# HarborC/PL-SLAM

Measured on NVIDIA H100. Metric: frames/sec (extract+match+pose-LM) 640x480, higher is better.
Workload: dtype u8/i32 front-end, f32 descriptors, f64 LM

## Files before the change

### pl-slam_b200/csrc/line.cu

```cuda

#include "common.cuh"
#include "lsd_grow_core.cuh"
#include "libm_glibc.cuh"
#include <math.h>
#include <string.h>
#include <stdlib.h>
#include <vector>
#include <algorithm>

namespace pl {

constexpr double kPI = 3.14159265358979323846;
constexpr double kDegToRads = kPI / 180;
constexpr int kBins = 1024;
constexpr int kChunkRows = 8;


struct PLKeyLineRec {
  float angle; int class_id; int octave; float ptx, pty; float response; float size;
  float startPointX, startPointY, endPointX, endPointY;
  float sPointInOctaveX, sPointInOctaveY, ePointInOctaveX, ePointInOctaveY;
  float lineLength; int numOfPixels;
};
static_assert(sizeof(PLKeyLineRec) == 68, "KeyLine layout");

struct LineParams {
  int w, h, sw, sh, npx;
  int nchunk;
  int s_th;
  int min_reg_size;
  int seg_cap, capL, nfeatures;
  double min_line_length;
  double prec, prec_hi, p, density_th;
  float sure_ca2, sure_cn2;
};

__device__ __forceinline__ float fast_atan2_deg_l(float y, float x) {
  const float k = (float)(180.0 / 3.14159265358979323846);
  const float p1 = 0.9997878412794807f * k, p3 = -0.3258083974640975f * k;
  const float p5 = 0.1555786518463281f * k, p7 = -0.04432655554792128f * k;
  const float eps = 2.220446049250313e-16f;
  const float ax = fabsf(x), ay = fabsf(y);
  const float c = __fdiv_rn(fminf(ax, ay), __fadd_rn(fmaxf(ax, ay), eps)), c2 = __fmul_rn(c, c);
  float a = __fmul_rn(__fadd_rn(__fmul_rn(__fadd_rn(__fmul_rn(__fadd_rn(__fmul_rn(p7, c2), p5), c2), p3), c2), p1), c);
  if (ax < ay) a = __fsub_rn(90.f, a);
  if (x < 0) a = __fsub_rn(180.f, a);
  if (y < 0) a = __fsub_rn(360.f, a);
  return a;
}
__device__ __forceinline__ double warp_max_d(double v) {
#pragma unroll
  for (int o = 16; o > 0; o >>= 1) v = fmax(v, __shfl_xor_sync(0xffffffffu, v, o));
  return v;
}
__device__ __forceinline__ double warp_min_d(double v) {
#pragma unroll
  for (int o = 16; o > 0; o >>= 1) v = fmin(v, __shfl_xor_sync(0xffffffffu, v, o));
  return v;
}

__global__ void __launch_bounds__(256) k_lsd_scale(LineParams P, const uint8_t* __restrict__ imgs, int stride,
                                                   long long frame_stride, uint8_t* __restrict__ scaled) {
  __shared__ uint8_t raw[44][48];
  __shared__ uint16_t hp[44][40];
  __shared__ uint8_t bl[40][40];
  const int tid = threadIdx.x;
  const int X0 = blockIdx.x * 32, Y0 = blockIdx.y * 32;
  const int bx0 = (5 * X0) >> 2, by0 = (5 * Y0) >> 2;
  const uint8_t* img = imgs + (long long)blockIdx.z * frame_stride;
  for (int i = tid; i < 44 * 44; i += 256) {
    int r = i / 44, c = i - r * 44;
    int gy = reflect101(min(by0 - 2 + r, 2 * P.h - 2), P.h), gx = reflect101(min(bx0 - 2 + c, 2 * P.w - 2), P.w);
    raw[r][c] = img[(long long)gy * stride + gx];
  }
  __syncthreads();
  for (int i = tid; i < 44 * 40; i += 256) {
    int r = i / 40, c = i - r * 40;
    const uint8_t* p = &raw[r][c];
    hp[r][c] = (uint16_t)(4 * (p[0] + p[4]) + 56 * (p[1] + p[3]) + 136 * p[2]);
  }
  __syncthreads();
  for (int i = tid; i < 40 * 40; i += 256) {
    int r = i / 40, c = i - r * 40;
    uint32_t s = 4u * (hp[r][c] + hp[r + 4][c]) + 56u * (hp[r + 1][c] + hp[r + 3][c]) + 136u * hp[r + 2][c];
    bl[r][c] = (uint8_t)((s + 32768u) >> 16);
  }
  __syncthreads();
  uint8_t* out = scaled + (long long)blockIdx.z * P.npx;
  for (int i = tid; i < 32 * 32; i += 256) {
    int ty = i >> 5, tx = i & 31;
    int x = X0 + tx, y = Y0 + ty;
    if (x >= P.sw || y >= P.sh) continue;
    int sx = (10 * x + 1) >> 3, xf = ((10 * x + 1) & 7) * 32;
    int sy = (10 * y + 1) >> 3, yf = ((10 * y + 1) & 7) * 32;
    if (sx >= P.w - 1) { sx = P.w - 1; xf = 0; }
    if (sy >= P.h - 1) { sy = P.h - 1; yf = 0; }
    int sx1 = min(sx + 1, P.w - 1), sy1 = min(sy + 1, P.h - 1);
    int lx = sx - bx0, lx1 = sx1 - bx0, ly = sy - by0, ly1 = sy1 - by0;
    int h0 = bl[ly][lx] * (256 - xf) + bl[ly][lx1] * xf;
    int h1 = bl[ly1][lx] * (256 - xf) + bl[ly1][lx1] * xf;
    out[(long long)y * P.sw + x] = (uint8_t)((h0 * (256 - yf) + h1 * yf + 32768) >> 16);
  }
}

constexpr float kNotDefDeg = -1024.f;
constexpr int kGradR = 510, kGradN = 2 * kGradR + 1;
struct GradRec { float deg, c, s, pad; };
__device__ __forceinline__ void grad_record(int gx, int gy, GradRec& rec, float2& scs) {
  const float deg = fast_atan2_deg_l((float)gx, (float)(-gy));
  const double af = (double)(float)((double)deg * kDegToRads);
  double sn, cs;
  sincos(af, &sn, &cs);
  rec.deg = deg; rec.c = (float)cs; rec.s = (float)sn; rec.pad = 0.f;
  const double ad = (double)deg * kDegToRads, dl = ad - af, h2 = 1.0 - 0.5 * dl * dl;
  scs = make_float2((float)(cs * h2 - sn * dl), (float)(sn * h2 + cs * dl));
}
__global__ void __launch_bounds__(256) k_lsd_grad_table(GradRec* __restrict__ T, float2* __restrict__ TS) {
  const int i = blockIdx.x * blockDim.x + threadIdx.x;
  if (i >= kGradN * kGradN) return;
  GradRec rec; float2 scs;
  grad_record(i / kGradN - kGradR, i % kGradN - kGradR, rec, scs);
  T[i] = rec; TS[i] = scs;
}
template <bool kVec>
__global__ void __launch_bounds__(256) k_lsd_grad(LineParams P, const uint8_t* __restrict__ scaled, const float4* __restrict__ T,
                                                  const float2* __restrict__ TS,
                                                  int4* __restrict__ REC, int* __restrict__ S2, float2* __restrict__ seedcs, int* __restrict__ maxs) {
  __shared__ int smax;
  if (threadIdx.x == 0) smax = 0;
  __syncthreads();
  const int x0 = (blockIdx.x * 64 + (threadIdx.x & 63)) * 4, y = blockIdx.y * 4 + (threadIdx.x >> 6);
  const int f = blockIdx.z;
  int smx = 0;
  if (x0 < P.sw && y < P.sh) {
    const uint8_t* S = scaled + (long long)f * P.npx + (long long)y * P.sw + x0;
    const bool lastrow = (y >= P.sh - 1);
    int r0[5], r1[5];
    if (kVec) {
      const unsigned w0 = *reinterpret_cast<const unsigned*>(S), w1 = lastrow ? 0u : *reinterpret_cast<const unsigned*>(S + P.sw);
#pragma unroll
      for (int k = 0; k < 4; k++) { r0[k] = (w0 >> (8 * k)) & 0xff; r1[k] = (w1 >> (8 * k)) & 0xff; }
      const bool in4 = (x0 + 4 < P.sw);
      r0[4] = in4 ? S[4] : 0; r1[4] = (in4 && !lastrow) ? S[P.sw + 4] : 0;
    } else {
#pragma unroll
      for (int k = 0; k < 5; k++) {
        const bool in = (x0 + k < P.sw);
        r0[k] = in ? S[k] : 0;
        r1[k] = (in && !lastrow) ? S[P.sw + k] : 0;
      }
    }
    int4 rec[4];
    float se[4][2];
    int sq[4];
#pragma unroll
    for (int k = 0; k < 4; k++) {
      rec[k] = make_int4(lg::kNotDef, __float_as_int(kNotDefDeg), 0, 0); se[k][0] = se[k][1] = 0.f; sq[k] = 0;
      if (x0 + k < P.sw - 1 && !lastrow) {
        const int DA = r1[k + 1] - r0[k], BC = r0[k + 1] - r1[k];
        const int gx = DA + BC, gy = DA - BC;
        const int s = gx * gx + gy * gy;
        sq[k] = s;
        if (s > P.s_th) {
          const int ti = (gx + kGradR) * kGradN + (gy + kGradR);
          const float4 t = __ldg(&T[ti]);
          const float2 scs = __ldg(&TS[ti]);
          rec[k] = make_int4(lg::kFree, __float_as_int(t.x), __float_as_int(t.y), __float_as_int(t.z));
          se[k][0] = scs.x; se[k][1] = scs.y;
          smx = max(smx, s);
        }
      }
    }
    const long long o = (long long)f * P.npx + (long long)y * P.sw + x0;
    if (kVec) {
#pragma unroll
      for (int k = 0; k < 4; k++) REC[o + k] = rec[k];
      *reinterpret_cast<int4*>(S2 + o) = make_int4(sq[0], sq[1], sq[2], sq[3]);
      float4* e4 = reinterpret_cast<float4*>(seedcs + o);
      e4[0] = make_float4(se[0][0], se[0][1], se[1][0], se[1][1]); e4[1] = make_float4(se[2][0], se[2][1], se[3][0], se[3][1]);
    } else {
      for (int k = 0; k < 4 && x0 + k < P.sw; k++) { REC[o + k] = rec[k]; S2[o + k] = sq[k]; seedcs[o + k] = make_float2(se[k][0], se[k][1]); }
    }
  }
#pragma unroll
  for (int o = 16; o > 0; o >>= 1) smx = max(smx, __shfl_xor_sync(0xffffffffu, smx, o));
  if ((threadIdx.x & 31) == 0 && smx > 0) atomicMax(&smax, smx);
  __syncthreads();
  if (threadIdx.x == 0 && smax > 0) atomicMax(&maxs[f], smax);
}
__device__ __forceinline__ double s_norm(int s) { return sqrt((double)s / 4.0); }
__device__ __forceinline__ int s_bin(int s, double bin_coef) { return (int)(s_norm(s) * bin_coef); }

__global__ void __launch_bounds__(256) k_lsd_hist(LineParams P, const int* __restrict__ S2, const int* __restrict__ maxs,
                                                  unsigned short* __restrict__ counts ) {
  __shared__ int hist[kBins];
  const int chunk = blockIdx.x, f = blockIdx.y, tid = threadIdx.x;
  for (int i = tid; i < kBins; i += 256) hist[i] = 0;
  __syncthreads();
  const int ms = maxs[f];
  const double max_grad = ms > 0 ? sqrt((double)ms / 4.0) : -1.0;
  const double bin_coef = (max_grad > 0) ? (double)(kBins - 1) / max_grad : 0.0;
  const int y0 = chunk * kChunkRows, y1 = min(y0 + kChunkRows, P.sh - 1);
  const int* SS = S2 + (long long)f * P.npx;
  for (int i = tid; i < (y1 - y0) * P.sw; i += 256) {
    int y = y0 + i / P.sw, x = i % P.sw;
    const int sv = SS[y * P.sw + x];
    if (sv > P.s_th) atomicAdd(&hist[s_bin(sv, bin_coef)], 1);
  }
  __syncthreads();
  for (int i = tid; i < kBins; i += 256) counts[((long long)f * kBins + i) * P.nchunk + chunk] = (unsigned short)hist[i];
}

__global__ void __launch_bounds__(kBins) k_lsd_scan(LineParams P, const unsigned short* __restrict__ counts,
                                                    int* __restrict__ offsets, int* __restrict__ ndef) {
  __shared__ int wsum[32];
  const int f = blockIdx.x, t = threadIdx.x, bin = kBins - 1 - t, lane = t & 31, wid = t >> 5;
  const unsigned short* c = counts + ((long long)f * kBins + bin) * P.nchunk;
  int tot = 0;
  for (int k = 0; k < P.nchunk; k++) tot += c[k];
  int incl = tot;
#pragma unroll
  for (int o = 1; o < 32; o <<= 1) { int v = __shfl_up_sync(0xffffffffu, incl, o); if (lane >= o) incl += v; }
  if (lane == 31) wsum[wid] = incl;
  __syncthreads();
  if (wid == 0) {
    int v = wsum[lane], in2 = v;
#pragma unroll
    for (int o = 1; o < 32; o <<= 1) { int u = __shfl_up_sync(0xffffffffu, in2, o); if (lane >= o) in2 += u; }
    wsum[lane] = in2 - v;
    if (lane == 31) ndef[f] = in2;
  }
  __syncthreads();
  int base = wsum[wid] + incl - tot;
  int* o = offsets + ((long long)f * kBins + bin) * P.nchunk;
  for (int k = 0; k < P.nchunk; k++) { o[k] = base; base += c[k]; }
}

__global__ void __launch_bounds__(128) k_lsd_scatter(LineParams P, const int* __restrict__ S2, const int* __restrict__ maxs,
                                                     const int* __restrict__ offsets, unsigned* __restrict__ order) {
  __shared__ unsigned short cnt[4][kBins];
  const int wid = threadIdx.x >> 5, lane = threadIdx.x & 31;
  const int chunk = blockIdx.x * 4 + wid, f = blockIdx.y;
  for (int i = lane; i < kBins; i += 32) cnt[wid][i] = 0;
  __syncwarp();
  if (chunk >= P.nchunk) return;
  const int ms = maxs[f];
  const double max_grad = ms > 0 ? sqrt((double)ms / 4.0) : -1.0;
  const double bin_coef = (max_grad > 0) ? (double)(kBins - 1) / max_grad : 0.0;
  const int y0 = chunk * kChunkRows, y1 = min(y0 + kChunkRows, P.sh - 1);
  const int* SS = S2 + (long long)f * P.npx;
  const int* off = offsets + (long long)f * kBins * P.nchunk;
  unsigned* O = order + (long long)f * P.npx;
  const int n = (y1 - y0) * P.sw;
  const unsigned lt = (1u << lane) - 1u;
  for (int i0 = 0; i0 < n; i0 += 32) {
    int i = i0 + lane, bin = -1, pix = 0;
    if (i < n) {
      int y = y0 + i / P.sw, x = i % P.sw;
      pix = x | (y << 16);
      const int sv = SS[y * P.sw + x];
      if (sv > P.s_th) bin = s_bin(sv, bin_coef);
    }
    unsigned peers = __match_any_sync(0xffffffffu, bin);
    if (bin >= 0) O[off[bin * P.nchunk + chunk] + cnt[wid][bin] + __popc(peers & lt)] = (unsigned)pix;
    __syncwarp();
    if (bin >= 0 && (peers & lt) == 0) cnt[wid][bin] += (unsigned short)__popc(peers);
    __syncwarp();
  }
}

constexpr int kGrowQ = 256;
constexpr int kCommitBatches = 4;
constexpr unsigned kGrowWatchdog = 6u * 1000u * 1000u;
__device__ __forceinline__ int first_zero(unsigned m) { return m == 0xffffffffu ? 32 : __ffs(~m) - 1; }

__device__ __forceinline__ void warp_commit(const lg::Params& GP, const lg::Frame& Fm, float4* __restrict__ segs, int lane) {
  using namespace lg;
  const unsigned lt = (1u << lane) - 1u;
  for (int round = 0; round < kCommitBatches; round++) {
    const int F = ld_i(&Fm.ctl[C_FIN]);
    if (F >= Fm.n) return;
    const int i = F + lane;
    const unsigned w1 = (i < Fm.n) ? ld_u(&Fm.st[i]) : 0u;
    const unsigned s1 = w1 & ST_STATE;
    const int pre1 = first_zero(__ballot_sync(0xffffffffu, s1 == ST_NOOP || s1 == ST_EATEN || s1 == ST_DONE));
    if (pre1 == 0) return;
    __threadfence();
    unsigned w2 = 0u;
    bool ok = false;
    if (lane < pre1) { w2 = ld_u(&Fm.st[i]); ok = task_valid(GP, Fm, i, w2); }
    const int pre2 = min(pre1, first_zero(__ballot_sync(0xffffffffu, ok)));
    float4 sg;
    const bool has = (lane < pre2) && task_has_segment(Fm, w2, sg);
    const unsigned ms = __ballot_sync(0xffffffffu, has);
    const int ns = ld_i(&Fm.ctl[C_NS]);
    if (has) { const int slot = ns + __popc(ms & lt); if (slot < GP.seg_cap) segs[slot] = sg; }
    __syncwarp();
    if (lane == 0) {
      st_i(&Fm.ctl[C_NS], ns + __popc(ms));
      __threadfence();
      a_max(&Fm.ctl[C_FIN], F + pre2);
    }
    if (pre2 < pre1) {
      const unsigned s2 = w2 & ST_STATE;
      if (lane == pre2 && (s2 == ST_DONE || s2 == ST_EATEN) &&
          (unsigned)a_cas(reinterpret_cast<int*>(&Fm.st[i]), (int)w2, (int)((w2 & ~(ST_STATE | ST_ABORT)) | ST_REDO)) == w2) {
        __threadfence();
        st_i(&Fm.ctl[C_REDO], i);
      }
      __syncwarp();
      return;
    }
    __syncwarp();
    if (pre2 < 32) return;
  }
}

template <int kWPC>
__global__ void __launch_bounds__(32 * kWPC) k_lsd_grow(LineParams P, lg::Params GP, int4* __restrict__ REC, const float2* __restrict__ seedcs,
                                                        const int* __restrict__ SQ, const unsigned* __restrict__ order, const int* __restrict__ ndef,
                                                        unsigned* __restrict__ ST, unsigned* __restrict__ POOL, int* __restrict__ CTL,
                                                        unsigned* __restrict__ LANEBUF, const double* __restrict__ wtab,
                                                        float4* __restrict__ segs, int* __restrict__ nseg, int* __restrict__ overflow,
                                                        int nframes, int wpf) {
  using namespace lg;
  __shared__ int wq_all[kWPC][kGrowQ];
  __shared__ unsigned ring_all[kWPC][32 * lg::kRing];
  const int lane = threadIdx.x & 31, wic = threadIdx.x >> 5;
  const long long gw = (long long)blockIdx.x * kWPC + wic;
  const int f = (int)(gw / wpf), wif = (int)(gw % wpf);
  if (f >= nframes) return;
  int* wq = wq_all[wic];
  Frame Fm;
  Fm.rec = REC + (long long)f * P.npx; Fm.seedcs = seedcs + (long long)f * P.npx; Fm.sq = SQ + (long long)f * P.npx;
  Fm.order = order + (long long)f * P.npx; Fm.n = ndef[f];
  Fm.st = ST + (long long)f * P.npx; Fm.pool = POOL + (long long)f * GP.pool_cap; Fm.ctl = CTL + (long long)f * kCtlStride; Fm.wtab = wtab;
  float4* S = segs + (long long)f * P.seg_cap;
  const bool solo = (wpf == 1);
  if (!solo && wif == 0) {
    for (unsigned iter = 0;; iter++) {
      __syncwarp();
      const int F = __shfl_sync(0xffffffffu, ld_i(&Fm.ctl[C_FIN]), 0);
      if (F >= Fm.n) break;
      if (iter > 4u * kGrowWatchdog) {
        if (lane == 0) { a_or(reinterpret_cast<unsigned*>(&Fm.ctl[C_ERR]), (unsigned)ERR_WATCHDOG); a_max(&Fm.ctl[C_FIN], Fm.n); }
        break;
      }
      warp_commit(GP, Fm, S, lane);
      if (__shfl_sync(0xffffffffu, ld_i(&Fm.ctl[C_FIN]), 0) == F) __nanosleep(200);
    }
    if (lane == 0) {
// ... 337 lines not shown
      if (gDL > 0) pgdL = __fadd_rn(pgdL, gDL); else ngdL = __fsub_rn(ngdL, gDL);
      if (gDO > 0) pgdO = __fadd_rn(pgdO, gDO); else ngdO = __fsub_rn(ngdO, gDO);
      sCorX = __fadd_rn(sCorX, dL0); sCorY = __fadd_rn(sCorY, dL1);
    }
    const float c = c_gaussG[hID];
    pgdL = __fmul_rn(c, pgdL); ngdL = __fmul_rn(c, ngdL); pgdO = __fmul_rn(c, pgdO); ngdO = __fmul_rn(c, ngdO);
    rs[hID][0] = pgdL; rs[hID][1] = ngdL; rs[hID][2] = __fmul_rn(pgdL, pgdL); rs[hID][3] = __fmul_rn(ngdL, ngdL);
    rs[hID][4] = pgdO; rs[hID][5] = ngdO; rs[hID][6] = __fmul_rn(pgdO, pgdO); rs[hID][7] = __fmul_rn(ngdO, ngdO);
  }
  __syncthreads();
  for (int a = tid; a < 72; a += 64) {
    const int q = a / 9, k = a - q * 9;
    const bool sq = (q == 2 || q == 3 || q == 6 || q == 7);
    float b = 0.f;
    for (int B = max(k - 1, 0); B <= min(k + 1, 8); B++) {
      const int off = (B - k + 1) * 7;
      for (int j = 0; j < 7; j++) {
        const float cg = s_gL[j + off], v = rs[B * 7 + j][q];
        b = __fadd_rn(b, sq ? __fmul_rn(__fmul_rn(cg, cg), v) : __fmul_rn(cg, v));
      }
    }
    band[q][k] = b;
  }
  __syncthreads();
  if (tid < 36) {
    const int bb = tid >> 2, c = tid & 3;
    const int qm = (c & 1) + ((c & 2) << 1), qs = qm + 2;
    const float invN = (bb == 0 || bb == 8) ? (float)(1.0 / (7 * 2.0)) : (float)(1.0 / (7 * 3.0));
    const float temp = __fmul_rn(band[qm][bb], invN);
    des[8 * bb + c] = temp;
    des[8 * bb + 4 + c] = sqrtf(__fsub_rn(__fmul_rn(band[qs][bb], invN), __fmul_rn(temp, temp)));
  }
  __syncthreads();
  if (tid == 0 || tid == 32) {
    const int k0 = tid ? 4 : 0;
    float acc = 0;
    for (int i = 0; i < 72; i += 8)
      for (int k = k0; k < k0 + 4; k++) acc = __fadd_rn(acc, __fmul_rn(des[i + k], des[i + k]));
    s_norm2[tid ? 1 : 0] = __fdiv_rn(1.f, sqrtf(acc));
  }
  __syncthreads();
  for (int i = tid; i < 72; i += 64) {
    float v = __fmul_rn(des[i], s_norm2[(i & 7) >> 2]);
    if ((double)v > 0.4) v = (float)0.4;
    des[i] = v;
  }
  __syncthreads();
  if (tid == 0) {
    float temp = 0;
    for (int i = 0; i < 72; i++) temp = __fadd_rn(temp, __fmul_rn(des[i], des[i]));
    s_norm2[0] = __fdiv_rn(1.f, sqrtf(temp));
  }
  __syncthreads();
  for (int i = tid; i < 72; i += 64) des[i] = __fmul_rn(des[i], s_norm2[0]);
  __syncthreads();
  if (tid < 32) {
    const float* f1 = &des[8 * c_comb[2 * tid]];
    const float* f2 = &des[8 * c_comb[2 * tid + 1]];
    unsigned r = 0;
#pragma unroll
    for (int i = 0; i < 8; i++) if (f1[i] > f2[i]) r += (1u << i);
    desc[((long long)f * P.capL + li) * 32 + tid] = (uint8_t)r;
  }
}

}

using namespace pl;

struct PLLine {
  PLLineConfig cfg;
  LineParams P;
  cudaStream_t stream = nullptr;
  uint8_t* d_scaled = nullptr;
  float2* d_seedcs = nullptr;
  lg::Params GP;
  int grow_warps_target = 132 * 16;
  int grow_wpf_max = 64;
  int grow_spec_max_batch = 0;
  size_t lane_warps = 0;
  int4* d_rec = nullptr; int* d_sq = nullptr;
  unsigned *d_st = nullptr, *d_pool = nullptr, *d_lanebuf = nullptr; int* d_ctl = nullptr; double* d_wtab = nullptr;
  GradRec* d_gtab = nullptr; float2* d_gtab_seed = nullptr;
  unsigned short* d_counts = nullptr;
  int *d_offsets = nullptr, *d_ndef = nullptr, *d_maxs = nullptr, *d_nseg = nullptr, *d_overflow = nullptr;
  unsigned* d_order = nullptr;
  float4* d_segs = nullptr;
  short2* d_dxy = nullptr;
  uint8_t* d_img = nullptr; PLKeyLineRec* d_kls = nullptr; uint8_t* d_desc = nullptr; double* d_lf = nullptr; int* d_nl = nullptr;
  uint8_t* d_mask = nullptr;
  size_t key_smem = 0;
  int last_B = 0;
  int timing = 0;
  cudaEvent_t ev0 = nullptr, ev1 = nullptr;
};

static const unsigned char h_comb[64] = {0, 1, 0, 2, 0, 3, 0, 4, 0, 5, 0, 6, 1, 2, 1, 3, 1, 4, 1, 5, 1, 6, 2, 3, 2, 4, 2, 5, 2, 6, 2, 7,
                                         2, 8, 3, 4, 3, 5, 3, 6, 3, 7, 3, 8, 4, 5, 4, 6, 4, 7, 4, 8, 5, 6, 5, 7, 5, 8, 6, 7, 6, 8, 7, 8};

extern "C" void pl_line_destroy(PLLine* h) {
  if (!h) return;
  cudaFree(h->d_gtab); cudaFree(h->d_gtab_seed); cudaFree(h->d_scaled); cudaFree(h->d_seedcs); cudaFree(h->d_rec); cudaFree(h->d_sq); cudaFree(h->d_st); cudaFree(h->d_pool); cudaFree(h->d_lanebuf); cudaFree(h->d_ctl); cudaFree(h->d_wtab); cudaFree(h->d_counts); cudaFree(h->d_offsets);
  cudaFree(h->d_ndef); cudaFree(h->d_maxs); cudaFree(h->d_nseg); cudaFree(h->d_overflow); cudaFree(h->d_order);
  cudaFree(h->d_segs); cudaFree(h->d_dxy); cudaFree(h->d_img); cudaFree(h->d_kls);
  cudaFree(h->d_desc); cudaFree(h->d_lf); cudaFree(h->d_nl); cudaFree(h->d_mask);
  if (h->stream) cudaStreamDestroy(h->stream);
  delete h;
}

extern "C" int pl_line_create(const PLLineConfig* cfg, PLLine** out) {
  PL_ARG(cfg && out);
  PL_ARG(cfg->width >= 64 && cfg->height >= 64 && cfg->width < 8000 && cfg->height < 8000 && cfg->nfeatures > 0 && cfg->max_batch >= 1);
  int rc = require_device();
  if (rc) return rc;
  PLLine* h = new PLLine;
  h->cfg = *cfg;
  LineParams& P = h->P;
  P.w = cfg->width; P.h = cfg->height;
  P.sw = (int)lrint(P.w * 0.8); P.sh = (int)lrint(P.h * 0.8);
  P.npx = P.sw * P.sh;
  P.nchunk = (P.sh - 1 + kChunkRows - 1) / kChunkRows;
  const double ANG_TH = 22.5, QUANT = 2.0;
  P.prec = kPI * ANG_TH / 180; P.p = ANG_TH / 180; P.density_th = 0.7;
  {
    const double twopi = 2 * kPI;
    double c = twopi - P.prec;
    while ((twopi - nextafter(c, 0.0)) <= P.prec) c = nextafter(c, 0.0);
    while (!((twopi - c) <= P.prec)) c = nextafter(c, 10.0);
    P.prec_hi = c;
  }
  {
    const double M = 0.05 * M_PI / 180.0, ca = cos(P.prec - M), cn = cos(P.prec + M);
    P.sure_ca2 = (float)(ca * ca); P.sure_cn2 = (float)(cn * cn);
  }
  const double rho = QUANT / sin(P.prec);
  int s = 0;
  while (sqrt((double)(s + 1) / 4.0) <= rho) s++;
  P.s_th = s;
  const double LOG_NT = 5 * (log10((double)P.sw) + log10((double)P.sh)) / 2 + log10(11.0);
  P.min_reg_size = (int)(size_t)(-LOG_NT / log10(P.p));
  P.seg_cap = cfg->segment_cap > 0 ? cfg->segment_cap : 8192;
  P.nfeatures = cfg->nfeatures; P.capL = cfg->nfeatures + 1; P.min_line_length = cfg->min_line_length;
  { size_t c2 = 1; while (c2 < (size_t)P.seg_cap) c2 <<= 1; h->key_smem = c2 * 8; }
  const size_t B = cfg->max_batch, npx = P.npx;
#define LN_TRY(e) do { int _r = (e); if (_r) { pl_line_destroy(h); return _r; } } while (0)
#define LN_CUDA(e) do { cudaError_t _e = (e); if (_e != cudaSuccess) { set_error("%s -> %s", #e, cudaGetErrorString(_e)); pl_line_destroy(h); return PL_ERR_CUDA; } } while (0)
  LN_CUDA(cudaStreamCreateWithFlags(&h->stream, cudaStreamNonBlocking));
  LN_TRY(dev_alloc(&h->d_scaled, npx * B)); LN_TRY(dev_alloc(&h->d_seedcs, npx * B)); LN_TRY(dev_alloc(&h->d_rec, npx * B));
  LN_TRY(dev_alloc(&h->d_sq, npx * B));
  {
    int dev = 0, sms = 132;
    cudaGetDevice(&dev); cudaDeviceGetAttribute(&sms, cudaDevAttrMultiProcessorCount, dev);
    h->grow_warps_target = sms * 16;
    if (const char* e = getenv("PLSLAM_LSD_GROW_WARPS")) { const int v = atoi(e); if (v > 0) h->grow_warps_target = v; }
    if (const char* e = getenv("PLSLAM_LSD_GROW_WPF")) { const int v = atoi(e); if (v > 0) h->grow_wpf_max = v; }
    if (const char* e = getenv("PLSLAM_LSD_GROW_SPEC_MAXB")) h->grow_spec_max_batch = atoi(e);
    lg::Params& G = h->GP;
    G.sw = P.sw; G.sh = P.sh; G.npx = P.npx; G.min_reg_size = P.min_reg_size; G.seg_cap = P.seg_cap;
    G.lane_cap = 1024; G.pool_cap = 4 * P.npx; G.window = 8192;
    if (const char* e = getenv("PLSLAM_LSD_GROW_WINDOW")) G.window = atoi(e);
    G.prec = P.prec; G.prec_hi = P.prec_hi; G.density_th = P.density_th;
    h->lane_warps = std::max<size_t>(std::min<size_t>(B * (size_t)h->grow_wpf_max, (size_t)h->grow_warps_target), B);
    LN_TRY(dev_alloc(&h->d_st, npx * B)); LN_TRY(dev_alloc(&h->d_pool, (size_t)G.pool_cap * B)); LN_TRY(dev_alloc(&h->d_ctl, (size_t)lg::kCtlStride * B));
    LN_TRY(dev_alloc(&h->d_lanebuf, h->lane_warps * 32 * (size_t)G.lane_cap));
    const int nw = 2 * kGradR * kGradR + 1;
    LN_TRY(dev_alloc(&h->d_wtab, (size_t)nw));
    k_lsd_wtab<<<(nw + 255) / 256, 256, 0, h->stream>>>(h->d_wtab, nw);
    LN_CUDA(cudaGetLastError());
    count_launch();
  }
  LN_TRY(dev_alloc(&h->d_counts, (size_t)kBins * P.nchunk * B)); LN_TRY(dev_alloc(&h->d_offsets, (size_t)kBins * P.nchunk * B));
  LN_TRY(dev_alloc(&h->d_ndef, B)); LN_TRY(dev_alloc(&h->d_maxs, B)); LN_TRY(dev_alloc(&h->d_nseg, B)); LN_TRY(dev_alloc(&h->d_overflow, 1));
  LN_TRY(dev_alloc(&h->d_order, npx * B)); LN_TRY(dev_alloc(&h->d_segs, (size_t)P.seg_cap * B));
  LN_TRY(dev_alloc(&h->d_dxy, (size_t)P.w * P.h * B));
  LN_CUDA(cudaMemset(h->d_overflow, 0, sizeof(int)));
  LN_TRY(dev_alloc(&h->d_gtab, (size_t)kGradN * kGradN)); LN_TRY(dev_alloc(&h->d_gtab_seed, (size_t)kGradN * kGradN));
  k_lsd_grad_table<<<(kGradN * kGradN + 255) / 256, 256, 0, h->stream>>>(h->d_gtab, h->d_gtab_seed);
  LN_CUDA(cudaGetLastError());
  LN_CUDA(cudaStreamSynchronize(h->stream));
  count_launch();
  {
    float gG[63], gL[21];
    double u = (7 * 3 - 1) / 2, sigma = (7 * 2 + 1) / 2, inv = -1 / (2 * sigma * sigma);
    for (int i = 0; i < 21; i++) { double d = i - u; gL[i] = (float)exp(d * d * inv); }
    u = (9 * 7 - 1) / 2; sigma = u; inv = -1 / (2 * sigma * sigma);
    for (int i = 0; i < 63; i++) { double d = i - u; gG[i] = (float)exp(d * d * inv); }
    LN_CUDA(cudaMemcpyToSymbol(c_gaussG, gG, sizeof(gG)));
    LN_CUDA(cudaMemcpyToSymbol(c_gaussL, gL, sizeof(gL)));
    LN_CUDA(cudaMemcpyToSymbol(c_comb, h_comb, sizeof(h_comb)));
  }
  LN_CUDA(cudaFuncSetAttribute(k_keylines, cudaFuncAttributeMaxDynamicSharedMemorySize, (int)h->key_smem));
  *out = h;
  return PL_OK;
}

extern "C" int pl_line_capacity(const PLLine* h) { return h ? h->P.capL : PL_ERR_ARG; }

extern "C" int pl_line_set_timing(PLLine* h, int on) {
  PL_ARG(h);
  if (on && !h->ev0) { PL_CUDA(cudaEventCreate(&h->ev0)); PL_CUDA(cudaEventCreate(&h->ev1)); }
  h->timing = on;
  return PL_OK;
}
extern "C" int pl_line_grow_ms(PLLine* h, float* ms) {
  PL_ARG(h && ms && h->ev0);
  PL_CUDA(cudaEventSynchronize(h->ev1));
  PL_CUDA(cudaEventElapsedTime(ms, h->ev0, h->ev1));
  return PL_OK;
}
extern "C" long long pl_line_grow_bytes_per_frame(const PLLine* h) { return h ? (long long)h->P.npx * 28 : 0; }

extern "C" int pl_line_extract_batch_dev(PLLine* h, const uint8_t* imgs, int stride, size_t frame_stride, int B,
                                         const uint8_t* mask, void* keylines, uint8_t* desc, double* linefunc, int* n,
                                         void* stream_) {
  PL_ARG(h && imgs && keylines && desc && linefunc && n && B >= 1 && B <= h->cfg.max_batch && stride >= h->cfg.width);
  cudaStream_t st = stream_ ? (cudaStream_t)stream_ : h->stream;
  const LineParams& P = h->P;
  h->last_B = B;
  PL_CUDA(cudaMemsetAsync(h->d_maxs, 0, sizeof(int) * B, st));
  k_lsd_scale<<<dim3((P.sw + 31) / 32, (P.sh + 31) / 32, B), 256, 0, st>>>(P, imgs, stride, (long long)frame_stride, h->d_scaled);
  PL_LAUNCH_CHECK();
  {
    const dim3 grd((P.sw + 255) / 256, (P.sh + 3) / 4, B);
    if (P.sw % 4 == 0)
      k_lsd_grad<true><<<grd, 256, 0, st>>>(P, h->d_scaled, reinterpret_cast<const float4*>(h->d_gtab), h->d_gtab_seed, h->d_rec, h->d_sq, h->d_seedcs, h->d_maxs);
    else
      k_lsd_grad<false><<<grd, 256, 0, st>>>(P, h->d_scaled, reinterpret_cast<const float4*>(h->d_gtab), h->d_gtab_seed, h->d_rec, h->d_sq, h->d_seedcs, h->d_maxs);
  }
  PL_LAUNCH_CHECK();
  k_lsd_hist<<<dim3(P.nchunk, B), 256, 0, st>>>(P, h->d_sq, h->d_maxs, h->d_counts);
  PL_LAUNCH_CHECK();
  k_lsd_scan<<<B, kBins, 0, st>>>(P, h->d_counts, h->d_offsets, h->d_ndef);
  PL_LAUNCH_CHECK();
  k_lsd_scatter<<<dim3((P.nchunk + 3) / 4, B), 128, 0, st>>>(P, h->d_sq, h->d_maxs, h->d_offsets, h->d_order);
  PL_LAUNCH_CHECK();
  if (B <= h->grow_spec_max_batch) {
    PL_CUDA(cudaMemsetAsync(h->d_st, 0, sizeof(unsigned) * (size_t)P.npx * B, st));
    k_lsd_grow_init<<<(B + 127) / 128, 128, 0, st>>>(h->d_ctl, B);
    PL_LAUNCH_CHECK();
    if (h->timing) PL_CUDA(cudaEventRecord(h->ev0, st));
    const int wpf = std::max(1, std::min(h->grow_wpf_max, h->grow_warps_target / B));
    k_lsd_grow<1><<<B * wpf, 32, 0, st>>>(P, h->GP, h->d_rec, h->d_seedcs, h->d_sq, h->d_order, h->d_ndef, h->d_st, h->d_pool, h->d_ctl,
                                          h->d_lanebuf, h->d_wtab, h->d_segs, h->d_nseg, h->d_overflow, B, wpf);
    PL_LAUNCH_CHECK();
  } else {
    if (h->timing) PL_CUDA(cudaEventRecord(h->ev0, st));
    static const int pre_maxb = getenv("PLSLAM_LSD_PRE_MAXB") ? atoi(getenv("PLSLAM_LSD_PRE_MAXB")) : 256;
    const int chunk = (int)std::min<long long>(B, 0xffffffffLL / P.npx);
    for (int b0 = 0; b0 < B; b0 += chunk) {
      const int nb = std::min(chunk, B - b0);
      const size_t po = (size_t)b0 * P.npx;
      if (B <= pre_maxb)
        k_lsd_grow_ordered<true><<<nb, 32, 0, st>>>(P, h->d_rec + po, h->d_sq + po, h->d_seedcs + po, h->d_order + po, h->d_ndef + b0,
                                                    h->d_pool + (size_t)b0 * h->GP.pool_cap, h->GP.pool_cap, h->d_st + po, h->d_wtab,
                                                    h->d_segs + (size_t)b0 * P.seg_cap, h->d_nseg + b0, h->d_overflow, nb);
      else
        k_lsd_grow_ordered<false><<<nb, 32, 0, st>>>(P, h->d_rec + po, h->d_sq + po, h->d_seedcs + po, h->d_order + po, h->d_ndef + b0,
                                                     h->d_pool + (size_t)b0 * h->GP.pool_cap, h->GP.pool_cap, h->d_st + po, h->d_wtab,
                                                     h->d_segs + (size_t)b0 * P.seg_cap, h->d_nseg + b0, h->d_overflow, nb);
    }
    PL_LAUNCH_CHECK();
  }
  if (h->timing) PL_CUDA(cudaEventRecord(h->ev1, st));
  k_keylines<<<B, 256, h->key_smem, st>>>(P, h->d_segs, h->d_nseg, mask, (PLKeyLineRec*)keylines, linefunc, n);
  PL_LAUNCH_CHECK();
  k_lbd_sobel<<<dim3((P.w + kSobOut - 1) / kSobOut, (P.h + kSobOut - 1) / kSobOut, B), 256, 0, st>>>(P, imgs, stride, (long long)frame_stride, h->d_dxy);
  PL_LAUNCH_CHECK();
  k_lbd_describe<<<dim3(P.capL, B), 64, 0, st>>>(P, (const PLKeyLineRec*)keylines, n, h->d_dxy, desc);
  PL_LAUNCH_CHECK();
  return PL_OK;
}

extern "C" int pl_line_check_overflow(PLLine* h) {
  PL_ARG(h);
  int ov = 0;
  PL_CUDA(cudaMemcpy(&ov, h->d_overflow, sizeof(int), cudaMemcpyDeviceToHost));
  if (ov) {
    cudaMemset(h->d_overflow, 0, sizeof(int));
    if (ov & 1) set_error("LSD produced more than segment_cap=%d segments", h->P.seg_cap);
    else set_error("LSD region growing gave a frame up (list pool of %d words exhausted, or watchdog): see pl_line_debug_ctl", h->GP.pool_cap);
    return PL_ERR_CAPACITY;
  }
  return PL_OK;
}

static int line_staging(PLLine* h) {
  if (h->d_img) return PL_OK;
  const size_t B = h->cfg.max_batch;
  int rc;
  if ((rc = dev_alloc(&h->d_img, (size_t)h->P.w * h->P.h * B))) return rc;
  if ((rc = dev_alloc(&h->d_kls, (size_t)h->P.capL * B))) return rc;
  if ((rc = dev_alloc(&h->d_desc, (size_t)h->P.capL * 32 * B))) return rc;
  if ((rc = dev_alloc(&h->d_lf, (size_t)h->P.capL * 3 * B))) return rc;
  if ((rc = dev_alloc(&h->d_nl, B))) return rc;
  if ((rc = dev_alloc(&h->d_mask, (size_t)h->P.w * h->P.h))) return rc;
  return PL_OK;
}

extern "C" int pl_line_extract_batch(PLLine* h, const uint8_t* imgs, int stride, size_t frame_stride, int B,
                                     const uint8_t* mask, void* keylines, uint8_t* desc, double* linefunc, int* n) {
  PL_ARG(h && imgs && keylines && desc && linefunc && n && B >= 1 && B <= h->cfg.max_batch && stride >= h->cfg.width);
  int rc = line_staging(h);
  if (rc) return rc;
  const int W = h->P.w, H = h->P.h;
  for (int b = 0; b < B; b++)
    PL_CUDA(cudaMemcpy2DAsync(h->d_img + (size_t)b * W * H, W, imgs + (size_t)b * frame_stride, stride, W, H, cudaMemcpyHostToDevice, h->stream));
  if (mask) PL_CUDA(cudaMemcpyAsync(h->d_mask, mask, (size_t)W * H, cudaMemcpyHostToDevice, h->stream));
  rc = pl_line_extract_batch_dev(h, h->d_img, W, (size_t)W * H, B, mask ? h->d_mask : nullptr, h->d_kls, h->d_desc, h->d_lf, h->d_nl, h->stream);
  if (rc) return rc;
  const size_t cap = h->P.capL;
  PL_CUDA(cudaMemcpyAsync(keylines, h->d_kls, cap * B * sizeof(PLKeyLineRec), cudaMemcpyDeviceToHost, h->stream));
  PL_CUDA(cudaMemcpyAsync(desc, h->d_desc, cap * B * 32, cudaMemcpyDeviceToHost, h->stream));
  PL_CUDA(cudaMemcpyAsync(linefunc, h->d_lf, cap * B * 3 * sizeof(double), cudaMemcpyDeviceToHost, h->stream));
  PL_CUDA(cudaMemcpyAsync(n, h->d_nl, (size_t)B * sizeof(int), cudaMemcpyDeviceToHost, h->stream));
  PL_CUDA(cudaStreamSynchronize(h->stream));
  return pl_line_check_overflow(h);
}
// ... 57 lines not shown
```

Before: 10050.

## Fuse LSD gradient, histogram, scan and scatter into one cluster kernel

Result: faster. 10750, median of 6 (+6.9%).

```diff
diff --git a/pl-slam_b200/csrc/line.cu b/pl-slam_b200/csrc/line.cu
--- a/pl-slam_b200/csrc/line.cu
+++ b/pl-slam_b200/csrc/line.cu
@@ -1,19 +1,21 @@
 
 #include "common.cuh"
+#include <cooperative_groups.h>
 #include "lsd_grow_core.cuh"
 #include "libm_glibc.cuh"
 #include <math.h>
 #include <string.h>
 #include <stdlib.h>
+#include <utility>
 #include <vector>
 #include <algorithm>
 
 namespace pl {
+namespace cg = cooperative_groups;
 
 constexpr double kPI = 3.14159265358979323846;
 constexpr double kDegToRads = kPI / 180;
 constexpr int kBins = 1024;
-constexpr int kChunkRows = 8;
 
 
 struct PLKeyLineRec {
@@ -26,7 +28,7 @@
 
 struct LineParams {
   int w, h, sw, sh, npx;
-  int nchunk;
+  int ord_cluster;
   int s_th;
   int min_reg_size;
   int seg_cap, capL, nfeatures;
@@ -122,17 +124,34 @@
   grad_record(i / kGradN - kGradR, i % kGradN - kGradR, rec, scs);
   T[i] = rec; TS[i] = scs;
 }
+__device__ __forceinline__ double s_norm(int s) { return sqrt((double)s / 4.0); }
+__device__ __forceinline__ int s_bin(int s, double bin_coef) { return (int)(s_norm(s) * bin_coef); }
+
+constexpr int kOrdThreads = 512, kOrdWarps = kOrdThreads / 32, kOrdBpt = kBins / kOrdThreads;
+constexpr int kOrdAhead = 3;
+constexpr size_t kOrdSmem = sizeof(int) * kOrdWarps * kBins;
+static_assert(kBins % kOrdThreads == 0, "the cluster scan gives every thread the same number of bins");
+
 template <bool kVec>
-__global__ void __launch_bounds__(256) k_lsd_grad(LineParams P, const uint8_t* __restrict__ scaled, const float4* __restrict__ T,
-                                                  const float2* __restrict__ TS,
-                                                  int4* __restrict__ REC, int* __restrict__ S2, float2* __restrict__ seedcs, int* __restrict__ maxs) {
-  __shared__ int smax;
-  if (threadIdx.x == 0) smax = 0;
-  __syncthreads();
-  const int x0 = (blockIdx.x * 64 + (threadIdx.x & 63)) * 4, y = blockIdx.y * 4 + (threadIdx.x >> 6);
-  const int f = blockIdx.z;
+__global__ void __launch_bounds__(kOrdThreads, 2) k_lsd_grad_order(LineParams P, const uint8_t* __restrict__ scaled,
+                                                                   const float4* __restrict__ T, const float2* __restrict__ TS,
+                                                                   int4* __restrict__ REC, int* S2, float2* __restrict__ seedcs,
+                                                                   unsigned* __restrict__ order, int* __restrict__ ndef) {
+  extern __shared__ int whist[];
+  __shared__ int ctot[kBins];
+  __shared__ int smax, wsum[kOrdWarps];
+  cg::cluster_group cl = cg::this_cluster();
+  const int C = (int)cl.num_blocks(), rank = (int)cl.block_rank();
+  const int f = blockIdx.x / C, tid = threadIdx.x, lane = tid & 31, wid = tid >> 5;
+  const int R = (P.sh + C - 1) / C, ys0 = min(P.sh, rank * R), ys1 = min(P.sh, ys0 + R);
+  for (int i = tid; i < kOrdWarps * kBins; i += kOrdThreads) whist[i] = 0;
+  if (tid == 0) smax = 0;
+  __syncthreads();
+
   int smx = 0;
-  if (x0 < P.sw && y < P.sh) {
+  const int qpr = (P.sw + 3) >> 2, nq = (ys1 - ys0) * qpr;
+  for (int q = tid; q < nq; q += kOrdThreads) {
+    const int yr = q / qpr, y = ys0 + yr, x0 = (q - yr * qpr) * 4;
     const uint8_t* S = scaled + (long long)f * P.npx + (long long)y * P.sw + x0;
     const bool lastrow = (y >= P.sh - 1);
     int r0[5], r1[5];
@@ -174,99 +193,101 @@
     const long long o = (long long)f * P.npx + (long long)y * P.sw + x0;
     if (kVec) {
 #pragma unroll
-      for (int k = 0; k < 4; k++) REC[o + k] = rec[k];
+      for (int k = 0; k < 4; k++) __stcs(&REC[o + k], rec[k]);
       *reinterpret_cast<int4*>(S2 + o) = make_int4(sq[0], sq[1], sq[2], sq[3]);
       float4* e4 = reinterpret_cast<float4*>(seedcs + o);
-      e4[0] = make_float4(se[0][0], se[0][1], se[1][0], se[1][1]); e4[1] = make_float4(se[2][0], se[2][1], se[3][0], se[3][1]);
+      __stcs(&e4[0], make_float4(se[0][0], se[0][1], se[1][0], se[1][1])); __stcs(&e4[1], make_float4(se[2][0], se[2][1], se[3][0], se[3][1]));
     } else {
-      for (int k = 0; k < 4 && x0 + k < P.sw; k++) { REC[o + k] = rec[k]; S2[o + k] = sq[k]; seedcs[o + k] = make_float2(se[k][0], se[k][1]); }
+      for (int k = 0; k < 4 && x0 + k < P.sw; k++) { __stcs(&REC[o + k], rec[k]); S2[o + k] = sq[k]; __stcs(&seedcs[o + k], make_float2(se[k][0], se[k][1])); }
     }
   }
 #pragma unroll
   for (int o = 16; o > 0; o >>= 1) smx = max(smx, __shfl_xor_sync(0xffffffffu, smx, o));
-  if ((threadIdx.x & 31) == 0 && smx > 0) atomicMax(&smax, smx);
-  __syncthreads();
-  if (threadIdx.x == 0 && smax > 0) atomicMax(&maxs[f], smax);
-}
-__device__ __forceinline__ double s_norm(int s) { return sqrt((double)s / 4.0); }
-__device__ __forceinline__ int s_bin(int s, double bin_coef) { return (int)(s_norm(s) * bin_coef); }
-
-__global__ void __launch_bounds__(256) k_lsd_hist(LineParams P, const int* __restrict__ S2, const int* __restrict__ maxs,
-                                                  unsigned short* __restrict__ counts ) {
-  __shared__ int hist[kBins];
-  const int chunk = blockIdx.x, f = blockIdx.y, tid = threadIdx.x;
-  for (int i = tid; i < kBins; i += 256) hist[i] = 0;
-  __syncthreads();
-  const int ms = maxs[f];
+  if (lane == 0 && smx > 0) atomicMax(&smax, smx);
+  cl.sync();
+
+  int ms = 0;
+  for (int r = 0; r < C; r++) ms = max(ms, *cl.map_shared_rank(&smax, r));
   const double max_grad = ms > 0 ? sqrt((double)ms / 4.0) : -1.0;
   const double bin_coef = (max_grad > 0) ? (double)(kBins - 1) / max_grad : 0.0;
-  const int y0 = chunk * kChunkRows, y1 = min(y0 + kChunkRows, P.sh - 1);
+
+  const int nr = max(0, min(ys1, P.sh - 1) - ys0);
+  const int wy0 = ys0 + wid * nr / kOrdWarps, wy1 = ys0 + (wid + 1) * nr / kOrdWarps;
   const int* SS = S2 + (long long)f * P.npx;
-  for (int i = tid; i < (y1 - y0) * P.sw; i += 256) {
-    int y = y0 + i / P.sw, x = i % P.sw;
-    const int sv = SS[y * P.sw + x];
-    if (sv > P.s_th) atomicAdd(&hist[s_bin(sv, bin_coef)], 1);
-  }
-  __syncthreads();
-  for (int i = tid; i < kBins; i += 256) counts[((long long)f * kBins + i) * P.nchunk + chunk] = (unsigned short)hist[i];
-}
-
-__global__ void __launch_bounds__(kBins) k_lsd_scan(LineParams P, const unsigned short* __restrict__ counts,
-                                                    int* __restrict__ offsets, int* __restrict__ ndef) {
-  __shared__ int wsum[32];
-  const int f = blockIdx.x, t = threadIdx.x, bin = kBins - 1 - t, lane = t & 31, wid = t >> 5;
-  const unsigned short* c = counts + ((long long)f * kBins + bin) * P.nchunk;
-  int tot = 0;
-  for (int k = 0; k < P.nchunk; k++) tot += c[k];
-  int incl = tot;
-#pragma unroll
-  for (int o = 1; o < 32; o <<= 1) { int v = __shfl_up_sync(0xffffffffu, incl, o); if (lane >= o) incl += v; }
+  int* hist = whist + wid * kBins;
+  for (int y = wy0; y < wy1; y++) {
+#pragma unroll 4
+    for (int x = lane; x < P.sw; x += 32) {
+      const int sv = SS[y * P.sw + x];
+      if (sv > P.s_th) atomicAdd(&hist[s_bin(sv, bin_coef)], 1);
+    }
+  }
+  __syncthreads();
+  for (int b = tid; b < kBins; b += kOrdThreads) {
+    int run = 0;
+#pragma unroll
+    for (int w = 0; w < kOrdWarps; w++) { const int c = whist[w * kBins + b]; whist[w * kBins + b] = run; run += c; }
+    ctot[b] = run;
+  }
+  cl.sync();
+  int a[kOrdBpt], p[kOrdBpt], tsum = 0;
+#pragma unroll
+  for (int j = 0; j < kOrdBpt; j++) a[j] = p[j] = 0;
+  for (int r = 0; r < C; r++) {
+    const int* rt = cl.map_shared_rank(ctot, r);
+#pragma unroll
+    for (int j = 0; j < kOrdBpt; j++) {
+      const int c = rt[kBins - 1 - tid * kOrdBpt - j];
+      a[j] += c;
+      if (r < rank) p[j] += c;
+    }
+  }
+  auto read_done = cl.barrier_arrive();
+#pragma unroll
+  for (int j = 0; j < kOrdBpt; j++) tsum += a[j];
+  int incl = tsum;
+#pragma unroll
+  for (int o = 1; o < 32; o <<= 1) { const int v = __shfl_up_sync(0xffffffffu, incl, o); if (lane >= o) incl += v; }
   if (lane == 31) wsum[wid] = incl;
   __syncthreads();
-  if (wid == 0) {
-    int v = wsum[lane], in2 = v;
-#pragma unroll
-    for (int o = 1; o < 32; o <<= 1) { int u = __shfl_up_sync(0xffffffffu, in2, o); if (lane >= o) in2 += u; }
-    wsum[lane] = in2 - v;
-    if (lane == 31) ndef[f] = in2;
-  }
-  __syncthreads();
-  int base = wsum[wid] + incl - tot;
-  int* o = offsets + ((long long)f * kBins + bin) * P.nchunk;
-  for (int k = 0; k < P.nchunk; k++) { o[k] = base; base += c[k]; }
-}
-
-__global__ void __launch_bounds__(128) k_lsd_scatter(LineParams P, const int* __restrict__ S2, const int* __restrict__ maxs,
-                                                     const int* __restrict__ offsets, unsigned* __restrict__ order) {
-  __shared__ unsigned short cnt[4][kBins];
-  const int wid = threadIdx.x >> 5, lane = threadIdx.x & 31;
-  const int chunk = blockIdx.x * 4 + wid, f = blockIdx.y;
-  for (int i = lane; i < kBins; i += 32) cnt[wid][i] = 0;
-  __syncwarp();
-  if (chunk >= P.nchunk) return;
-  const int ms = maxs[f];
-  const double max_grad = ms > 0 ? sqrt((double)ms / 4.0) : -1.0;
-  const double bin_coef = (max_grad > 0) ? (double)(kBins - 1) / max_grad : 0.0;
-  const int y0 = chunk * kChunkRows, y1 = min(y0 + kChunkRows, P.sh - 1);
-  const int* SS = S2 + (long long)f * P.npx;
-  const int* off = offsets + (long long)f * kBins * P.nchunk;
+  int e = incl - tsum;
+#pragma unroll
+  for (int w = 0; w < kOrdWarps; w++) e += (w < wid) ? wsum[w] : 0;
+  if (rank == 0 && tid == kOrdThreads - 1) ndef[f] = e + tsum;
+#pragma unroll
+  for (int j = 0; j < kOrdBpt; j++) {
+    const int b = kBins - 1 - tid * kOrdBpt - j;
+#pragma unroll
+    for (int w = 0; w < kOrdWarps; w++) whist[w * kBins + b] += e + p[j];
+    e += a[j];
+  }
+  __syncthreads();
+
   unsigned* O = order + (long long)f * P.npx;
-  const int n = (y1 - y0) * P.sw;
   const unsigned lt = (1u << lane) - 1u;
-  for (int i0 = 0; i0 < n; i0 += 32) {
-    int i = i0 + lane, bin = -1, pix = 0;
-    if (i < n) {
-      int y = y0 + i / P.sw, x = i % P.sw;
-      pix = x | (y << 16);
-      const int sv = SS[y * P.sw + x];
-      if (sv > P.s_th) bin = s_bin(sv, bin_coef);
-    }
-    unsigned peers = __match_any_sync(0xffffffffu, bin);
-    if (bin >= 0) O[off[bin * P.nchunk + chunk] + cnt[wid][bin] + __popc(peers & lt)] = (unsigned)pix;
-    __syncwarp();
-    if (bin >= 0 && (peers & lt) == 0) cnt[wid][bin] += (unsigned short)__popc(peers);
-    __syncwarp();
-  }
+  int y = wy0, x0 = 0;
+  while (y < wy1) {
+    int sv[kOrdAhead];
+    unsigned pk[kOrdAhead];
+#pragma unroll
+    for (int u = 0; u < kOrdAhead; u++) {
+      const int x = x0 + lane;
+      pk[u] = (unsigned)(x | (y << 16));
+      sv[u] = (y < wy1 && x < P.sw) ? SS[y * P.sw + x] : 0;
+      x0 += 32;
+      if (x0 >= P.sw) { x0 = 0; y++; }
+    }
+#pragma unroll
+    for (int u = 0; u < kOrdAhead; u++) {
+      const int bin = (sv[u] > P.s_th) ? s_bin(sv[u], bin_coef) : -1;
+      const unsigned peers = __match_any_sync(0xffffffffu, bin);
+      if (bin >= 0) __stcs(&O[hist[bin] + __popc(peers & lt)], pk[u]);
+      __syncwarp();
+      if (bin >= 0 && (peers & lt) == 0) hist[bin] += __popc(peers);
+      __syncwarp();
+    }
+  }
+  cl.barrier_wait(std::move(read_done));
 }
 
 constexpr int kGrowQ = 256;
@@ -770,8 +791,7 @@
   int4* d_rec = nullptr; int* d_sq = nullptr;
   unsigned *d_st = nullptr, *d_pool = nullptr, *d_lanebuf = nullptr; int* d_ctl = nullptr; double* d_wtab = nullptr;
   GradRec* d_gtab = nullptr; float2* d_gtab_seed = nullptr;
-  unsigned short* d_counts = nullptr;
-  int *d_offsets = nullptr, *d_ndef = nullptr, *d_maxs = nullptr, *d_nseg = nullptr, *d_overflow = nullptr;
+  int *d_ndef = nullptr, *d_nseg = nullptr, *d_overflow = nullptr;
   unsigned* d_order = nullptr;
   float4* d_segs = nullptr;
   short2* d_dxy = nullptr;
@@ -788,8 +808,8 @@
 
 extern "C" void pl_line_destroy(PLLine* h) {
   if (!h) return;
-  cudaFree(h->d_gtab); cudaFree(h->d_gtab_seed); cudaFree(h->d_scaled); cudaFree(h->d_seedcs); cudaFree(h->d_rec); cudaFree(h->d_sq); cudaFree(h->d_st); cudaFree(h->d_pool); cudaFree(h->d_lanebuf); cudaFree(h->d_ctl); cudaFree(h->d_wtab); cudaFree(h->d_counts); cudaFree(h->d_offsets);
-  cudaFree(h->d_ndef); cudaFree(h->d_maxs); cudaFree(h->d_nseg); cudaFree(h->d_overflow); cudaFree(h->d_order);
+  cudaFree(h->d_gtab); cudaFree(h->d_gtab_seed); cudaFree(h->d_scaled); cudaFree(h->d_seedcs); cudaFree(h->d_rec); cudaFree(h->d_sq); cudaFree(h->d_st); cudaFree(h->d_pool); cudaFree(h->d_lanebuf); cudaFree(h->d_ctl); cudaFree(h->d_wtab);
+  cudaFree(h->d_ndef); cudaFree(h->d_nseg); cudaFree(h->d_overflow); cudaFree(h->d_order);
   cudaFree(h->d_segs); cudaFree(h->d_dxy); cudaFree(h->d_img); cudaFree(h->d_kls);
   cudaFree(h->d_desc); cudaFree(h->d_lf); cudaFree(h->d_nl); cudaFree(h->d_mask);
   if (h->stream) cudaStreamDestroy(h->stream);
@@ -807,7 +827,7 @@
   P.w = cfg->width; P.h = cfg->height;
   P.sw = (int)lrint(P.w * 0.8); P.sh = (int)lrint(P.h * 0.8);
   P.npx = P.sw * P.sh;
-  P.nchunk = (P.sh - 1 + kChunkRows - 1) / kChunkRows;
+  P.ord_cluster = std::max(1, std::min(8, P.sh / 8));
   const double ANG_TH = 22.5, QUANT = 2.0;
   P.prec = kPI * ANG_TH / 180; P.p = ANG_TH / 180; P.density_th = 0.7;
   {
@@ -857,8 +877,7 @@
     LN_CUDA(cudaGetLastError());
     count_launch();
   }
-  LN_TRY(dev_alloc(&h->d_counts, (size_t)kBins * P.nchunk * B)); LN_TRY(dev_alloc(&h->d_offsets, (size_t)kBins * P.nchunk * B));
-  LN_TRY(dev_alloc(&h->d_ndef, B)); LN_TRY(dev_alloc(&h->d_maxs, B)); LN_TRY(dev_alloc(&h->d_nseg, B)); LN_TRY(dev_alloc(&h->d_overflow, 1));
+  LN_TRY(dev_alloc(&h->d_ndef, B)); LN_TRY(dev_alloc(&h->d_nseg, B)); LN_TRY(dev_alloc(&h->d_overflow, 1));
   LN_TRY(dev_alloc(&h->d_order, npx * B)); LN_TRY(dev_alloc(&h->d_segs, (size_t)P.seg_cap * B));
   LN_TRY(dev_alloc(&h->d_dxy, (size_t)P.w * P.h * B));
   LN_CUDA(cudaMemset(h->d_overflow, 0, sizeof(int)));
@@ -878,6 +897,8 @@
     LN_CUDA(cudaMemcpyToSymbol(c_comb, h_comb, sizeof(h_comb)));
   }
   LN_CUDA(cudaFuncSetAttribute(k_keylines, cudaFuncAttributeMaxDynamicSharedMemorySize, (int)h->key_smem));
+  LN_CUDA(cudaFuncSetAttribute(k_lsd_grad_order<true>, cudaFuncAttributeMaxDynamicSharedMemorySize, (int)kOrdSmem));
+  LN_CUDA(cudaFuncSetAttribute(k_lsd_grad_order<false>, cudaFuncAttributeMaxDynamicSharedMemorySize, (int)kOrdSmem));
   *out = h;
   return PL_OK;
 }
@@ -905,22 +926,23 @@
   cudaStream_t st = stream_ ? (cudaStream_t)stream_ : h->stream;
   const LineParams& P = h->P;
   h->last_B = B;
-  PL_CUDA(cudaMemsetAsync(h->d_maxs, 0, sizeof(int) * B, st));
   k_lsd_scale<<<dim3((P.sw + 31) / 32, (P.sh + 31) / 32, B), 256, 0, st>>>(P, imgs, stride, (long long)frame_stride, h->d_scaled);
   PL_LAUNCH_CHECK();
   {
-    const dim3 grd((P.sw + 255) / 256, (P.sh + 3) / 4, B);
+    cudaLaunchConfig_t lc = {};
+    lc.gridDim = dim3((unsigned)(P.ord_cluster * B)); lc.blockDim = dim3(kOrdThreads); lc.dynamicSmemBytes = kOrdSmem; lc.stream = st;
+    cudaLaunchAttribute at;
+    at.id = cudaLaunchAttributeClusterDimension;
+    at.val.clusterDim.x = P.ord_cluster; at.val.clusterDim.y = 1; at.val.clusterDim.z = 1;
+    lc.attrs = &at; lc.numAttrs = 1;
+    const float4* T = reinterpret_cast<const float4*>(h->d_gtab);
     if (P.sw % 4 == 0)
-      k_lsd_grad<true><<<grd, 256, 0, st>>>(P, h->d_scaled, reinterpret_cast<const float4*>(h->d_gtab), h->d_gtab_seed, h->d_rec, h->d_sq, h->d_seedcs, h->d_maxs);
+      PL_CUDA(cudaLaunchKernelEx(&lc, k_lsd_grad_order<true>, P, (const uint8_t*)h->d_scaled, T, (const float2*)h->d_gtab_seed,
+                                 h->d_rec, h->d_sq, h->d_seedcs, h->d_order, h->d_ndef));
     else
-      k_lsd_grad<false><<<grd, 256, 0, st>>>(P, h->d_scaled, reinterpret_cast<const float4*>(h->d_gtab), h->d_gtab_seed, h->d_rec, h->d_sq, h->d_seedcs, h->d_maxs);
-  }
-  PL_LAUNCH_CHECK();
-  k_lsd_hist<<<dim3(P.nchunk, B), 256, 0, st>>>(P, h->d_sq, h->d_maxs, h->d_counts);
-  PL_LAUNCH_CHECK();
-  k_lsd_scan<<<B, kBins, 0, st>>>(P, h->d_counts, h->d_offsets, h->d_ndef);
-  PL_LAUNCH_CHECK();
-  k_lsd_scatter<<<dim3((P.nchunk + 3) / 4, B), 128, 0, st>>>(P, h->d_sq, h->d_maxs, h->d_offsets, h->d_order);
+      PL_CUDA(cudaLaunchKernelEx(&lc, k_lsd_grad_order<false>, P, (const uint8_t*)h->d_scaled, T, (const float2*)h->d_gtab_seed,
+                                 h->d_rec, h->d_sq, h->d_seedcs, h->d_order, h->d_ndef));
+  }
   PL_LAUNCH_CHECK();
   if (B <= h->grow_spec_max_batch) {
     PL_CUDA(cudaMemsetAsync(h->d_st, 0, sizeof(unsigned) * (size_t)P.npx * B, st));
```
